# mir-group/pair_allegro

Measured on AMD Instinct MI355X. Metric: atom_steps_per_sec, higher is better.
Workload: dtype f32-equivalent (f16x2 split on the f16 matrix cores, f32 accumulate); 1 GPU; BASELINE config 4: 1000000-atom bulk Si (50^3 diamond cells), model S (l_max=1, U=32, S=64, 2 layers), r_max 5.0 A + skin 1.0 A, NVE dt=1 fs; grid=1x1x1, rebuilds=4, comm=serial, comm_transport=library/hosted/single-rank gather-scatter

## Files before the change

### pair_allegro_amd/csrc/fused.hip

```cpp
#include <hip/hip_runtime.h>

#include <cmath>
#include <algorithm>
#include <cstdio>
#include <cstdlib>
#include <cstring>
#include <type_traits>

#include "../../include/allegro_hip.h"
#include "engine.h"
#define AHIP_RING 4
#include "fused_common.h"
#include "fused_h.h"
#include "prims.h"

#ifndef AHIP_FUSED_PART
#define AHIP_FUSED_PART 0
#endif
namespace ahip {


[[maybe_unused]] static constexpr int MAX_TILE_SLOTS = 128;
static constexpr int MAXNL = 3;
static constexpr int STG_LD = 132;
// ... 23 lines not shown
  double *f, *eatom, *partial;
  long long *prof;
  float *dbg;
  float cp[6];
  int *err;
  double *vatom;
};

template <int NW, int NL = MAXNL> struct __attribute__((aligned(16))) Lds {
  static constexpr int SLOTS = 16 * NW;
  static constexpr int MAXA = NW == 4 ? 6 : 12;
  float stage[SLOTS * STG_LD];
  float env[NL][MAXA * ENV_LD];
  float denv[MAXA * ENV_LD];
  float tp[NL][5 * 32];
  float park[NW][8 * ROW];
  double eacc[MAXA];
  double virw[NW][6];
  int aoff[2][MAXA + 2];
  float rc[16];
  float scale[16], shift[16];
  float res[NL][2];
  int chunk[2];
};


__device__ __host__ constexpr int R_Z1TB() { return 0; }
__device__ __host__ constexpr int R_Z2TB() { return 4; }
__device__ __host__ constexpr int R_U0() { return 8; }
__device__ __host__ constexpr int R_W0() { return 12; }
__device__ __host__ constexpr int R_LSZ(int MD) { return 16 + 4 * MD; }
__device__ __host__ constexpr int R_LAYER(int kk, int MD = 2) { return 16 + R_LSZ(MD) * kk; }
__device__ __host__ constexpr int R_TOTAL(int NL, int MD = 2) { return 16 + R_LSZ(MD) * NL; }

static constexpr float C_S3 = 1.7320508075688772f;
static constexpr float C_P1 = 0.5773502691896258f;
static constexpr float C_P4 = 0.7071067811865476f;

typedef __bf16 bf16x8 __attribute__((ext_vector_type(8)));
struct Bop { u32x4 hi, mid, lo; };

__device__ __forceinline__ f32x4 mfma_b(u32x4 a, u32x4 b, f32x4 c) {
  return __builtin_amdgcn_mfma_f32_16x16x32_bf16(__builtin_bit_cast(bf16x8, a), __builtin_bit_cast(bf16x8, b), c, 0, 0, 0);
}
__device__ __forceinline__ void split2(float v0, float v1, unsigned &hi, unsigned &mid, unsigned &lo) {
  const unsigned a = __builtin_bit_cast(unsigned, v0), b = __builtin_bit_cast(unsigned, v1);
// ... 96 lines not shown
  const int fidx = tid & 127;
  for (int a = tid >> 7; a < na; a += NW / 2) {
    const int s0 = aoff[a], s1 = aoff[a + 1];
    float acc0 = 0.f, acc1 = 0.f, acc2 = 0.f, acc3 = 0.f;
    int sl = s0;
    for (; sl + 4 <= s1; sl += 4) {
      acc0 += lds.stage[sl * STG_LD + fidx];
      acc1 += lds.stage[(sl + 1) * STG_LD + fidx];
      acc2 += lds.stage[(sl + 2) * STG_LD + fidx];
      acc3 += lds.stage[(sl + 3) * STG_LD + fidx];
    }
    for (; sl < s1; ++sl) acc0 += lds.stage[sl * STG_LD + fidx];
    dst[a * ENV_LD + fidx] = scale * ((acc0 + acc1) + (acc2 + acc3));
  }
}
enum { PH_GEOM = 0, PH_TB, PH_EMB, PH_ENV, PH_TP, PH_MIX, PH_LAT, PH_OUT, PH_BLAT, PH_BMIX, PH_BTP, PH_BENV, PH_BEMB, PH_BTB, PH_FIN, PH_N };
#define PHASE(id) do { if (PROF) { long long _t = clock64(); pacc[id] += _t - tprev; tprev = _t; } } while (0)

template <int AR> struct RingT {
  int act = 1;
  f32x4 f[AR != 0 ? 1 : RING];
  u32x4 b[AR == 0 ? 1 : (AR == 1 ? RINGB : AR == 2 ? RINGB2 : RINGH)];
};
template <int AR, int KT, int NT, bool ACC, int RPI, class Epi>
__device__ __forceinline__ void lin(__amdgpu_buffer_rsrc_t W, int &wp, const f32x4 (&in)[KT], f32x4 (&out)[NT], int v16, RingT<AR> &ring, Epi epi) {
  if (!ring.act) {
    if constexpr (!ACC) {
#pragma unroll
      for (int t = 0; t < NT; ++t) out[t] = f32x4{0.f, 0.f, 0.f, 0.f};
    }
    return;
  }
  if constexpr (AR == 3) {
    static_assert(KT % 2 == 0, "K-steps are pairs of 16-feature tiles");
    Hop b[1][KT / 2], unused[1][NT / 2];
#pragma unroll
    for (int ks = 0; ks < KT / 2; ++ks) b[0][ks] = split_pair_h(in[2 * ks], in[2 * ks + 1]);
    Epi ep[1] = {epi};
    linear_h<1, KT / 2, NT, ACC, false, (4 * RPI) % RINGH, Epi>(W, wp, b, reinterpret_cast<f32x4 (&)[1][NT]>(out), unused, v16, ring.b, ep);
  } else if constexpr (AR != 0) {
    static_assert(KT % 2 == 0, "K-steps are pairs of 16-feature tiles");
    constexpr int NTERM = AR == 1 ? 3 : 2;
    Bop b[KT / 2], unused[NT / 2];
#pragma unroll
    for (int ks = 0; ks < KT / 2; ++ks) b[ks] = split_pair(in[2 * ks], in[2 * ks + 1]);
    linear_b<KT / 2, NT, ACC, false, (2 * NTERM * RPI) % RingB<NTERM>::N, Epi, NTERM>(W, wp, b, out, unused, v16, ring.b, epi);
  } else {
    linear_s<KT, NT, ACC, (4 * RPI) % RING, Epi>(W, wp, in, out, v16, ring.f, epi);
  }
}

template <int RPI, class Epi>
__device__ __forceinline__ void lin_m3(__amdgpu_buffer_rsrc_t W, int &wp, const f32x4 (&in0)[2], const f32x4 (&in1)[2], const f32x4 (&in2)[2], f32x4 (&out)[3][2], int v16,
                                       RingT<3> &ring, Epi (&epi)[3]) {
  if (!ring.act) {
#pragma unroll
    for (int q = 0; q < 3; ++q) { out[q][0] = f32x4{0.f, 0.f, 0.f, 0.f}; out[q][1] = f32x4{0.f, 0.f, 0.f, 0.f}; }
    return;
  }
  Hop b[3][1], unused[3][1];
  b[0][0] = split_pair_h(in0[0], in0[1]); b[1][0] = split_pair_h(in1[0], in1[1]); b[2][0] = split_pair_h(in2[0], in2[1]);
  linear_h<3, 1, 2, false, false, (4 * RPI) % RINGH, Epi>(W, wp, b, out, unused, v16, ring.b, epi);
}

struct TileIn {
  int a0, a1, e0, e1;
  float rx, ry, rz;
  int eii, jat, tt;
  int eoff;
};
__device__ __forceinline__ void tile_fetch(const FusedArgs &A, int tile, int ntiles, int s, int tid, TileIn &n) {
  n.a0 = n.a1 = n.e0 = n.e1 = 0;
  n.rx = 1.f; n.ry = 0.f; n.rz = 0.f;
  n.eii = 0; n.jat = 0; n.tt = 0; n.eoff = 0;
  if (tile >= ntiles) return;
  n.a0 = A.tile_a0[tile]; n.a1 = A.tile_a0[tile + 1]; n.e0 = A.tile_e0[tile]; n.e1 = A.tile_e0[tile + 1];
  const int e = n.e0 + s, na = n.a1 - n.a0;
  if (e < n.e1) {
    n.rx = A.rvec[3 * (size_t)e]; n.ry = A.rvec[3 * (size_t)e + 1]; n.rz = A.rvec[3 * (size_t)e + 2];
    n.eii = A.e_ii[e];
    n.jat = A.e_j[e];
    n.tt = A.e_tt[e];
  }
  if (tid <= na) n.eoff = A.eoff[n.a0 + tid];
}

template <int NW, bool PROF, int AR, bool TBT, int NLT, int MD = 2, bool VA = false, int RD = 1>
__global__ void __launch_bounds__(NW * 64, 2) k_fused(FusedArgs A) {
  constexpr int NTHREADS = NW * 64, MAXA = Lds<NW>::MAXA;
  constexpr bool SAVEZ = AR == 3;
  constexpr bool PARKV = true;
  constexpr bool STGROWS = true;
  constexpr int OZL = 4 + 4 * (MD - 1), OU = 4 + 4 * MD, OVIN = 8 + 4 * MD;
  static_assert(MD >= 1 && MD <= 3 && (MD == 2 || (AR == 3 && TBT)), "latent MLP depth 1 / 3: f16x2 instances with the two-body table only");
  static_assert(RD == 1 || (RD == 2 && AR == 3 && TBT && !PROF), "read-out depth 2: f16x2 instances with the two-body table only, not profiled");
  __shared__ Lds<NW, NLT> lds;
  const int tid = threadIdx.x, lane = tid & 63, j = lane & 15, g = lane >> 4, wave = tid >> 6;
  const int v16 = lane * 16;
  __amdgpu_buffer_rsrc_t SB, WB;
  {
    unsigned long long b = (unsigned long long)(A.scratch + (size_t)blockIdx.x * A.wg_scratch + (size_t)wave * A.wave_scratch);
    unsigned lo = __builtin_amdgcn_readfirstlane((unsigned)b), hi = __builtin_amdgcn_readfirstlane((unsigned)(b >> 32));
    SB = __builtin_amdgcn_make_buffer_rsrc((void *)(((unsigned long long)hi << 32) | lo), 0, (int)(A.wave_scratch * 4), 0x00020000);
    WB = __builtin_amdgcn_make_buffer_rsrc((void *)A.wbase, 0, A.wbytes, 0x00020000);
  }
  if (A.maxdeg_sel && ((*A.maxdeg_sel <= 64) != (NW == 4))) return;
  const float *__restrict__ Wb = A.wbase;
// ... 2 lines not shown
    lds.tp[k / 160][k % 160] = Wb[A.o_tpl + k] * (pth == 1 ? C_P1 : pth == 4 ? C_P4 : 1.f);
  }
  const int ntiles = *A.ntiles;
  constexpr int NL = NLT;
  double acc_part = 0.0;
  long long pacc[PH_N];
  long long tprev = 0;
  const long long t_clk0 = clock64(), t_wall0 = wall_clock64();
  if (PROF) {
#pragma unroll
    for (int k = 0; k < PH_N; ++k) pacc[k] = 0;
    tprev = clock64();
  }
  float *const pk = lds.park[wave];
  RingT<AR> ring;
  int wp = A.o_stream;
  if constexpr (AR != 0) ring_prime_b(WB, wp, v16, ring.b);
  else ring_prime(WB, wp, v16, ring.f);
  if (tid < MAXA) lds.eacc[tid] = 0.0;
  if (lane < 6) lds.virw[wave][lane] = 0.0;
  if (A.T <= 4 && tid < A.T * A.T) lds.rc[tid] = (float)A.rcut[tid];
  if (tid < A.T) { lds.scale[tid] = Wb[A.o_scale + tid]; lds.shift[tid] = Wb[A.o_shift + tid]; }
  if (tid < 2 * A.NL) lds.res[tid >> 1][tid & 1] = Wb[A.o_res[tid >> 1] + (tid & 1)];

  const int s = wave * 16 + j;
  float *const st = lds.stage + s * STG_LD;
  if (tid == 0) lds.chunk[0] = (int)atomicAdd(A.tile_counter, (unsigned)A.tchunk);
  __syncthreads();
  int par = 0, cpar = 0, ck = 0;
  int cbase = __builtin_amdgcn_readfirstlane(lds.chunk[0]);

  TileIn nx_;
  tile_fetch(A, cbase, ntiles, s, tid, nx_);

  for (;;) {
    const int tile = cbase + ck;
    if (tile >= ntiles) break;
    int claimed = 0;
    if (ck == 0 && tid == 0) claimed = (int)atomicAdd(A.tile_counter, (unsigned)A.tchunk);
    const int a0 = nx_.a0, a1 = nx_.a1, e0 = nx_.e0, e1 = nx_.e1;
    const int wact = __builtin_amdgcn_readfirstlane(e0 + wave * 16 < e1 ? 1 : 0);
    ring.act = wact;
    const int v16t = wact ? v16 : 0x7ffffff0;
    const int na = a1 - a0;
    par ^= 1;
    int *const aoffp = lds.aoff[par];
    const int e = e0 + s;
    const bool valid = e < e1;
    const float rx = nx_.rx, ry = nx_.ry, rz = nx_.rz;
    const int aloc = valid ? nx_.eii - a0 : 0, jat = nx_.jat, ti = nx_.tt >> 4, tj = nx_.tt & 15;
    if (tid <= na) aoffp[tid] = nx_.eoff - e0;
    const float d = sqrtf(rx * rx + ry * ry + rz * rz);
    const float inv = 1.f / d;
    const float nx = rx * inv, ny = ry * inv, nz = rz * inv;
    const float rc = A.T <= 4 ? lds.rc[ti * A.T + tj] : (float)A.rcut[ti * A.T + tj];
    const float xx = d / rc;
    float fc, dfc_dx;
    cutoff_poly_c(A.p, A.cp, xx, fc, dfc_dx);
    if (!valid) { fc = 0.f; dfc_dx = 0.f; }
    const float Y1 = C_S3 * ny, Y2 = C_S3 * nz, Y3 = C_S3 * nx;
    const float pref = 2.f / rc;
    const float PI = 3.14159265358979323846f;
    const float *const envrow = lds.env[0] + aloc * ENV_LD;
    const float *const denvrow = lds.denv + aloc * ENV_LD;
    PHASE(PH_GEOM);

    f32x4 x[4];
    float tb_t = 0.f, tb_invh = 0.f;
    if constexpr (TBT) {
      tb_invh = (float)A.tb_nk / rc;
      const float sft = d * tb_invh;
      const int kq = min((int)sft, A.tb_nk - 1);
// ... 16 lines not shown
      {
        const float *pt = Wb + A.o_pair + (size_t)(ti * A.T + tj) * 64;
#pragma unroll
        for (int t = 0; t < 4; ++t) z[t] = *(const f32x4 *)(pt + 16 * t + 4 * g);
      }
      f32x4 bfin[2];
#pragma unroll
      for (int r = 0; r < 4; ++r) {
        const float n = (float)(4 * g + r + 1);
        bfin[0][r] = g < 2 ? pref * __builtin_amdgcn_sinf(0.5f * n * xx) * inv * fc : 0.f;
        bfin[1][r] = 0.f;
      }
      lin<AR, 2, 4, true, 0>(WB, wp, bfin, z, v16t, ring, EpiSiluSaveD{SB, R_Z1TB(), v16t});
      lin<AR, 4, 4, false, 0>(WB, wp, z, z2, v16t, ring, EpiSiluSaveD{SB, R_Z2TB(), v16t});
      lin<AR, 4, 4, false, 0>(WB, wp, z2, x, v16t, ring, EpiSaveScale{{SB, R_U0(), v16t}, fc});
    }
    PHASE(PH_TB);
    {
      f32x4 w0[4];
      lin<AR, 4, 4, false, 0>(WB, wp, x, w0, v16t, ring, EpiSavePark{{SB, R_W0(), v16t}, pk, 0, lane});
    }
    if (ck == 0 && tid == 0) lds.chunk[cpar ^ 1] = claimed;
    __syncthreads();
    PHASE(PH_EMB);

    f32x4 zr[2];
#pragma unroll
    for (int kk = 0; kk < NL; ++kk) {
      const bool last = (kk == NL - 1);
      const int RL = R_LAYER(kk, MD);
      float *const envk = lds.env[0] + kk * (MAXA * ENV_LD);
      f32x4 V[4][2];
      {
        f32x4 om[4];
        lin<AR, 4, 4, false, 0>(WB, wp, x, om, v16t, ring, EpiSaveFrom2{{SB, RL + 0, v16t}});
#pragma unroll
        for (int t = 0; t < 2; ++t) {
          float *sp = st + 16 * t + 4 * g;
          *(f32x4 *)(sp) = om[t];
          *(f32x4 *)(sp + 32) = om[2 + t] * Y1;
          *(f32x4 *)(sp + 64) = om[2 + t] * Y2;
          *(f32x4 *)(sp + 96) = om[2 + t] * Y3;
        }
        __syncthreads();
        reduce_stage(lds, aoffp, envk, na, A.cenv, tid);
        __syncthreads();
// ... 20 lines not shown
#pragma unroll
        for (int t = 0; t < 2; ++t) {
          const int b = 16 * t + 4 * g;
          const f32x4 e0v = *(const f32x4 *)(en + b), e1v = *(const f32x4 *)(en + 32 + b), e2v = *(const f32x4 *)(en + 64 + b),
                      e3v = *(const f32x4 *)(en + 96 + b);
          const f32x4 v0 = V[0][t], v1 = V[1][t], v2 = V[2][t], v3 = V[3][t];
          Vp[0][t] = *(const f32x4 *)(tp + b) * v0 * e0v + *(const f32x4 *)(tp + 32 + b) * (v1 * e1v + v2 * e2v + v3 * e3v);
          if (!last) {
            const f32x4 p2 = *(const f32x4 *)(tp + 64 + b), p3 = *(const f32x4 *)(tp + 96 + b), c4 = *(const f32x4 *)(tp + 128 + b);
            const f32x4 p2v0 = p2 * v0, p3e0 = p3 * e0v;
            Vp[1][t] = p2v0 * e1v + p3e0 * v1 + c4 * (v2 * e3v - v3 * e2v);
            Vp[2][t] = p2v0 * e2v + p3e0 * v2 + c4 * (v3 * e1v - v1 * e3v);
            Vp[3][t] = p2v0 * e3v + p3e0 * v3 + c4 * (v1 * e2v - v2 * e1v);
          }
          __builtin_amdgcn_sched_barrier(0);
        }
      }
      PHASE(PH_TP);
      if (!last) {
        f32x4 o2[2];
        if constexpr (AR == 3) {
          f32x4 o3[3][2];
          if (PARKV && kk + 1 == NL - 1) {
            lin<AR, 2, 2, false, 0>(WB, wp, Vp[0], o2, v16t, ring, EpiPark{pk, 0, lane});
            EpiPark ep[3] = {EpiPark{pk, 2, lane}, EpiPark{pk, 4, lane}, EpiPark{pk, 6, lane}};
            lin_m3<1>(WB, wp, Vp[1], Vp[2], Vp[3], o3, v16t, ring, ep);
          } else {
            lin<AR, 2, 2, false, 0>(WB, wp, Vp[0], o2, v16t, ring, EpiSavePark{{SB, R_LAYER(kk + 1, MD) + OVIN + 0, v16t}, pk, 0, lane});
            EpiSavePark ep[3] = {EpiSavePark{{SB, R_LAYER(kk + 1, MD) + OVIN + 2, v16t}, pk, 2, lane}, EpiSavePark{{SB, R_LAYER(kk + 1, MD) + OVIN + 4, v16t}, pk, 4, lane},
                                 EpiSavePark{{SB, R_LAYER(kk + 1, MD) + OVIN + 6, v16t}, pk, 6, lane}};
            lin_m3<1>(WB, wp, Vp[1], Vp[2], Vp[3], o3, v16t, ring, ep);
          }
        } else if (PARKV && kk + 1 == NL - 1) {
          lin<AR, 2, 2, false, 0>(WB, wp, Vp[0], o2, v16t, ring, EpiPark{pk, 0, lane});
          lin<AR, 2, 2, false, 1>(WB, wp, Vp[1], o2, v16t, ring, EpiPark{pk, 2, lane});
          lin<AR, 2, 2, false, 2>(WB, wp, Vp[2], o2, v16t, ring, EpiPark{pk, 4, lane});
          lin<AR, 2, 2, false, 3>(WB, wp, Vp[3], o2, v16t, ring, EpiPark{pk, 6, lane});
        } else {
          lin<AR, 2, 2, false, 0>(WB, wp, Vp[0], o2, v16t, ring, EpiSavePark{{SB, R_LAYER(kk + 1, MD) + OVIN + 0, v16t}, pk, 0, lane});
          lin<AR, 2, 2, false, 1>(WB, wp, Vp[1], o2, v16t, ring, EpiSavePark{{SB, R_LAYER(kk + 1, MD) + OVIN + 2, v16t}, pk, 2, lane});
          lin<AR, 2, 2, false, 2>(WB, wp, Vp[2], o2, v16t, ring, EpiSavePark{{SB, R_LAYER(kk + 1, MD) + OVIN + 4, v16t}, pk, 4, lane});
          lin<AR, 2, 2, false, 3>(WB, wp, Vp[3], o2, v16t, ring, EpiSavePark{{SB, R_LAYER(kk + 1, MD) + OVIN + 6, v16t}, pk, 6, lane});
        }
      }
      PHASE(PH_MIX);
      {
        f32x4 cat[6], z[4], z2[4];
        cat[0] = x[0]; cat[1] = x[1]; cat[2] = x[2]; cat[3] = x[3]; cat[4] = Vp[0][0]; cat[5] = Vp[0][1];
        const bool stg = STGROWS && last;
        float *const sq = st + 4 * g;
#define AHIP_HIDDEN(KT, IN, OUT, H) do { \
          if (stg && (H) >= MD - 1) { \
            if (SAVEZ && (H) == MD) lin<AR, KT, 4, false, 0>(WB, wp, IN, OUT, v16t, ring, EpiSiluSaveZL{sq, 4}); \
            else lin<AR, KT, 4, false, 0>(WB, wp, IN, OUT, v16t, ring, EpiSiluSaveDL{sq, (H) == MD ? 4 : 0}); \
// ... 18 lines not shown
          zr[0] = ra * za[0] + rbf * up[0]; zr[1] = ra * za[1] + rbf * up[1];
        }
      }
      PHASE(PH_LAT);
    }

    f32x4 upre[4], zt[4], w0h[2];
#pragma unroll
    for (int t = 0; t < 2; ++t) if (!SAVEZ) upre[t] = bload(SB, v16t, (R_LAYER(NL - 1, MD) + OU + t) * ROW * 4);
    if (!STGROWS) load_rows<4>(SB, R_LAYER(NL - 1, MD) + OZL, zt, v16t);
    __builtin_amdgcn_sched_barrier(0);
    f32x4 zr2[2];
    if constexpr (RD == 2) {
      f32x4 hr[2];
#pragma unroll
      for (int t = 0; t < 2; ++t)
#pragma unroll
        for (int r = 0; r < 4; ++r) hr[t][r] = silu1(zr[t][r]);
      lin<AR, 2, 2, false, 0>(WB, wp, hr, zr2, v16t, ring, EpiNone{});
    }
    f32x4 (&zo)[2] = RD == 2 ? zr2 : zr;
    f32x4 wo1[2];
#pragma unroll
    for (int t = 0; t < 2; ++t) wo1[t] = *(const f32x4 *)(Wb + A.o_out1 + 16 * t + 4 * g);
    float eps = 0.f;
#pragma unroll
    for (int t = 0; t < 2; ++t)
#pragma unroll
      for (int r = 0; r < 4; ++r) eps += silu1(zo[t][r]) * wo1[t][r];
    eps = gsum(eps);
    asm volatile("" : "+v"(eps));

    float bsc = 1.f;
    if constexpr (AR == 3) {
      int bex;
      (void)frexpf(lds.scale[ti] * A.cenv, &bex);
      bex = min(max(bex, -100), 100);
      bsc = ldexpf(1.f, -bex);
      if (g == 0) st[128] = ldexpf(1.f, bex);
    }
    const float deps = valid ? lds.scale[ti] * A.cenv * bsc : 0.f;
    f32x4 dx[4];
    f32x4 dzr[2];
#pragma unroll
    for (int t = 0; t < 2; ++t)
#pragma unroll
      for (int r = 0; r < 4; ++r) dzr[t][r] = deps * wo1[t][r] * dsilu1(zo[t][r]);
// ... 93 lines not shown
        for (int t = 0; t < 4; ++t) dx[t] += dcat[t];
        dVp[0][0] = dcat[4]; dVp[0][1] = dcat[5];
      }
      if (kk == 0) {
#pragma unroll
        for (int t = 0; t < 2; ++t) {
          Vk[0][t] = W0b[t];
          Vk[1][t] = W0b[2 + t] * Y1; Vk[2][t] = W0b[2 + t] * Y2; Vk[3][t] = W0b[2 + t] * Y3;
        }
      }
      if (PARKV && last && kk > 0) {
#pragma unroll
        for (int lm = 0; lm < 4; ++lm)
#pragma unroll
          for (int t = 0; t < 2; ++t) Vk[lm][t] = park_load(pk, 2 * lm + t, lane);
      }
      f32x4 om1[2];
      load_rows<2>(SB, RL + 2, om1, v16t);
      __builtin_amdgcn_sched_barrier(0);
      PHASE(PH_BLAT);
      if (!last) {
        f32x4 in2[2], o2[2];
        in2[0] = park_load(pk, 0, lane); in2[1] = park_load(pk, 1, lane);
        lin<AR, 2, 2, false, 0>(WB, wp, in2, o2, v16t, ring, EpiNone{});
        dVp[0][0] += o2[0]; dVp[0][1] += o2[1];
        if constexpr (AR == 3) {
          f32x4 i1[2] = {park_load(pk, 2, lane), park_load(pk, 3, lane)}, i2[2] = {park_load(pk, 4, lane), park_load(pk, 5, lane)},
                i3[2] = {park_load(pk, 6, lane), park_load(pk, 7, lane)};
          f32x4 o3[3][2];
          EpiNone ep[3];
          lin_m3<1>(WB, wp, i1, i2, i3, o3, v16t, ring, ep);
#pragma unroll
          for (int q = 0; q < 3; ++q) { dVp[1 + q][0] = o3[q][0]; dVp[1 + q][1] = o3[q][1]; }
        } else {
          in2[0] = park_load(pk, 2, lane); in2[1] = park_load(pk, 3, lane);
          lin<AR, 2, 2, false, 1>(WB, wp, in2, dVp[1], v16t, ring, EpiNone{});
          in2[0] = park_load(pk, 4, lane); in2[1] = park_load(pk, 5, lane);
          lin<AR, 2, 2, false, 2>(WB, wp, in2, dVp[2], v16t, ring, EpiNone{});
          in2[0] = park_load(pk, 6, lane); in2[1] = park_load(pk, 7, lane);
          lin<AR, 2, 2, false, 3>(WB, wp, in2, dVp[3], v16t, ring, EpiNone{});
        }
      }
      __builtin_amdgcn_sched_barrier(0);
      PHASE(PH_BMIX);
      {
        const float *en = envrow + kk * (MAXA * ENV_LD);
        const float *tp = lds.tp[kk];
#pragma unroll
        for (int t = 0; t < 2; ++t) {
          const int b = 16 * t + 4 * g;
          const f32x4 e0v = *(const f32x4 *)(en + b), e1v = *(const f32x4 *)(en + 32 + b), e2v = *(const f32x4 *)(en + 64 + b),
                      e3v = *(const f32x4 *)(en + 96 + b);
          const f32x4 v0 = Vk[0][t], v1 = Vk[1][t], v2 = Vk[2][t], v3 = Vk[3][t];
          const f32x4 g0 = dVp[0][t];
          const f32x4 q0 = *(const f32x4 *)(tp + b) * g0, q1 = *(const f32x4 *)(tp + 32 + b) * g0;
          f32x4 a0v = q0 * e0v, a1v = q1 * e1v, a2v = q1 * e2v, a3v = q1 * e3v;
          f32x4 b0v = q0 * v0, b1v = q1 * v1, b2v = q1 * v2, b3v = q1 * v3;
// ... 33 lines not shown
                      d3 = *(const f32x4 *)(denvrow + 96 + b);
          dom[t] = d0;
          dom[2 + t] = d1 * Y1 + d2 * Y2 + d3 * Y3;
          const f32x4 p1 = d1 * om1[t], p2 = d2 * om1[t], p3 = d3 * om1[t];
          dY1 += (p1[0] + p1[1]) + (p1[2] + p1[3]); dY2 += (p2[0] + p2[1]) + (p2[2] + p2[3]); dY3 += (p3[0] + p3[1]) + (p3[2] + p3[3]);
          __builtin_amdgcn_sched_barrier(0);
        }
        asm volatile("" : "+v"(dY1), "+v"(dY2), "+v"(dY3));
        if (kk > 0) {
          if (!SAVEZ) load_rows<4>(SB, R_LAYER(kk - 1, MD) + OU, upre, v16t);
          load_rows<4>(SB, R_LAYER(kk - 1, MD) + OZL, zt, v16t);
        } else {
          if constexpr (!TBT) {
            load_rows<4>(SB, R_U0(), upre, v16t);
            load_rows<4>(SB, R_Z2TB(), zt, v16t);
          } else load_rows<4>(SB, R_Z1TB(), zt, v16t);
          load_rows<2>(SB, R_W0() + 2, w0h, v16t);
        }
        __builtin_amdgcn_sched_barrier(0);
        lin<AR, 4, 4, true, 0>(WB, wp, dom, dx, v16t, ring, EpiNone{});
      }
      PHASE(PH_BENV);
    }
    {
      const int ntile = (ck + 1 == A.tchunk) ? __builtin_amdgcn_readfirstlane(lds.chunk[cpar ^ 1]) : tile + 1;
      tile_fetch(A, ntile, ntiles, s, tid, nx_);
    }
    f32x4 zt1b[4];
    if constexpr (!TBT) load_rows<4>(SB, R_Z1TB(), zt1b, v16t);
    __builtin_amdgcn_sched_barrier(0);
    {
      f32x4 dw0[4];
#pragma unroll
      for (int t = 0; t < 2; ++t) {
        const f32x4 d0 = park_load(pk, 0 + t, lane), d1 = park_load(pk, 2 + t, lane), d2 = park_load(pk, 4 + t, lane), d3 = park_load(pk, 6 + t, lane);
        dw0[t] = d0;
        dw0[2 + t] = d1 * Y1 + d2 * Y2 + d3 * Y3;
#pragma unroll
        for (int r = 0; r < 4; ++r) { dY1 += d1[r] * w0h[t][r]; dY2 += d2[r] * w0h[t][r]; dY3 += d3[r] * w0h[t][r]; }
      }
      asm volatile("" : "+v"(dY1), "+v"(dY2), "+v"(dY3));
      lin<AR, 4, 4, true, 0>(WB, wp, dw0, dx, v16t, ring, EpiNone{});
      if constexpr (TBT) wp = A.o_stream;
    }
    PHASE(PH_BEMB);
    float dd_part = 0.f;
    if constexpr (TBT) {
      f32x4 accv = dx[0] * zt[0];
#pragma unroll
      for (int t = 1; t < 4; ++t) accv += dx[t] * zt[t];
// ... 24 lines not shown
    }
    PHASE(PH_BTB);
    {
      const float ibs = AR == 3 ? st[128] : 1.f;
      const float dfc_tot = gsum(dfc_part) * ibs;
      const float dd = dfc_tot * (dfc_dx / rc) + gsum(dd_part) * ibs;
      const float y1 = gsum(dY1) * ibs, y2 = gsum(dY2) * ibs, y3 = gsum(dY3) * ibs;
      const float Gx = C_S3 * y3, Gy = C_S3 * y1, Gz = C_S3 * y2;
      float rxe = rx, rye = ry, rze = rz;
      asm volatile("" : "+v"(rxe), "+v"(rye), "+v"(rze));
      const float inve = 1.f / sqrtf(rxe * rxe + rye * rye + rze * rze);
      const float nxe = rxe * inve, nye = rye * inve, nze = rze * inve;
      const float gn = Gx * nxe + Gy * nye + Gz * nze;
      const float gx = dd * nxe + (Gx - gn * nxe) * inve;
      const float gy = dd * nye + (Gy - gn * nye) * inve;
      const float gz = dd * nze + (Gz - gn * nze) * inve;
      if (A.dbg && valid && g == 0) {
        float *dp = A.dbg + 8 * (size_t)e;
        dp[0] = gx; dp[1] = gy; dp[2] = gz; dp[3] = dd; dp[4] = dfc_tot; dp[5] = y1; dp[6] = y2; dp[7] = y3;
      }
#if !defined(ABL_NOW) && !defined(ABL_NOROWS) && !defined(ABL_NOROWLD) && !defined(ABL_NOROWST)
      if (AR == 3 && valid && !(fabsf(gx) + fabsf(gy) + fabsf(gz) + fabsf(eps) < 3.0e38f)) *A.err = 1;
#endif
      if (g == 0) {
        st[0] = valid ? gx : 0.f; st[1] = valid ? gy : 0.f; st[2] = valid ? gz : 0.f; st[3] = valid ? eps : 0.f;
        if (valid) {
#ifndef ABL_NOATOM
          atomicAdd(&A.f[3 * (size_t)jat], -(double)gx);
          atomicAdd(&A.f[3 * (size_t)jat + 1], -(double)gy);
          atomicAdd(&A.f[3 * (size_t)jat + 2], -(double)gz);
#endif
        }
      }
      float w6[6] = {-rx * gx, -ry * gy, -rz * gz, -0.5f * (rx * gy + ry * gx), -0.5f * (rx * gz + rz * gx), -0.5f * (ry * gz + rz * gy)};
#pragma unroll
      for (int c = 0; c < 6; ++c) w6[c] = valid ? w6[c] : 0.f;
#pragma unroll
      for (int c = 0; c < 6; ++c) {
#pragma unroll
        for (int off = 8; off > 0; off >>= 1) w6[c] += __shfl_xor(w6[c], off, 64);
      }
      if (lane < 6) {
        const float mine = lane == 0 ? w6[0] : lane == 1 ? w6[1] : lane == 2 ? w6[2] : lane == 3 ? w6[3] : lane == 4 ? w6[4] : w6[5];
        lds.virw[wave][lane] += (double)mine;
      }
      if constexpr (VA) vatom_scatter(A.vatom, jat, g, valid, rx, ry, rz, gx, gy, gz);
    }
    int tidf = tid;
    asm volatile("" : "+v"(tidf));
    const int caf = tidf >> 4;
    int2 cil = make_int2(0, 0);
    if (caf < na) cil = A.centre[a0 + caf];
    __syncthreads();
    {
      const int col = tidf & 3, part = (tidf >> 2) & 3;
      float sum = 0.f;
      if (caf < na)
        for (int sl = aoffp[caf] + part; sl < aoffp[caf + 1]; sl += 4) sum += lds.stage[sl * STG_LD + col];
      sum += __shfl_xor(sum, 4, 64);
      sum += __shfl_xor(sum, 8, 64);
      if (caf < na && part == 0) {
        if (col < 3) atomicAdd(&A.f[3 * (size_t)cil.x + col], (double)sum);
        else {
          const float ei = lds.scale[cil.y] * (sum * A.cenv) + lds.shift[cil.y];
          if (A.eatom) A.eatom[cil.x] = (double)ei;
          lds.eacc[caf] += (double)ei;
        }
      }
    }
    PHASE(PH_FIN);
    if (++ck == A.tchunk) { ck = 0; cpar ^= 1; cbase = __builtin_amdgcn_readfirstlane(lds.chunk[cpar]); }
  }
  __syncthreads();
  if (tid == 0) {
    for (int a = 0; a < MAXA; ++a) acc_part += lds.eacc[a];
  } else if (tid >= 64 && tid < 70) {
    for (int w = 0; w < NW; ++w) acc_part += lds.virw[w][tid - 64];
  }
  if (PROF && lane == 0) {
#pragma unroll
    for (int k = 0; k < PH_N; ++k) atomicAdd((unsigned long long *)&A.prof[k], (unsigned long long)pacc[k]);
  }
  if (A.prof && tid == 0) {
    long long *o = A.prof + PH_N + 4 * (size_t)blockIdx.x;
    o[0] = clock64() - t_clk0;
    o[1] = t_wall0;
    o[2] = wall_clock64();
    o[3] = ((long long)__builtin_amdgcn_s_getreg((20 << 0) | (0 << 6) | (31 << 11)) << 32) | (unsigned)__builtin_amdgcn_s_getreg((4 << 0) | (0 << 6) | (31 << 11));
  }
  if (tid == 0) A.partial[7 * (size_t)blockIdx.x] = acc_part;
  if (tid >= 64 && tid < 70) A.partial[7 * (size_t)blockIdx.x + 1 + (tid - 64)] = acc_part;
}


void fused_launch_bf16(int nw, bool prof, int arith, bool tbt, int grid, hipStream_t s, const FusedArgs &A);
void fused_launch_f16(int nw, bool prof, int md, int grid, hipStream_t s, const FusedArgs &A);
void fused_launch_f16_rd2(int nw, int md, int grid, hipStream_t s, const FusedArgs &A);
#if AHIP_FUSED_PART == 3
void fused_launch_f16_rd2(int nw, int md, int grid, hipStream_t s, const FusedArgs &A) {
  dispatch<Choices<4, 8>, Choices<1, 2, 3>, Choices<1, 3, 2>, Choices<VAR_VA, VAR_PLAIN>>([&](auto nw, auto nl, auto md, auto var) {
    hipLaunchKernelGGL((k_fused<nw, false, 3, true, nl, md, var == VAR_VA, 2>), dim3(grid), dim3(nw * 64), 0, s, A);
  }, nw, A.NL, md, fused_variant(A.vatom, false));
}
#endif
#if AHIP_FUSED_PART == 2
void fused_launch_f16(int nw, bool prof, int md, int grid, hipStream_t s, const FusedArgs &A) {
#ifdef AHIP_ASM_ONLY
#ifndef AHIP_ASM_NW
#define AHIP_ASM_NW 4
#endif
  hipLaunchKernelGGL((k_fused<AHIP_ASM_NW, false, 3, true, 2, 2>), dim3(grid), dim3(AHIP_ASM_NW * 64), 0, s, A);
#else
  dispatch<Choices<4, 8>, Choices<1, 2, 3>, Choices<1, 3, 2>, Variants>([&](auto nw, auto nl, auto md, auto var) {
    if constexpr (var != VAR_PROF || md == 2) hipLaunchKernelGGL((k_fused<nw, var == VAR_PROF, 3, true, nl, md, var == VAR_VA>), dim3(grid), dim3(nw * 64), 0, s, A);
// ... 422 lines not shown
```

### pair_allegro_amd/csrc/fused_h.h

```cpp
#pragma once
#include <cstring>

#include "fused_common.h"

namespace ahip {

typedef _Float16 f16x2 __attribute__((ext_vector_type(2)));
typedef _Float16 f16x8 __attribute__((ext_vector_type(8)));
typedef float f32x2 __attribute__((ext_vector_type(2)));
struct Hop { u32x4 hi, lo; };
static constexpr float H_LO_SCALE = 2048.f, H_LO_INV = 1.f / 2048.f;
static constexpr int RINGH = 8;

__device__ __forceinline__ f32x4 mfma_h(u32x4 a, u32x4 b, f32x4 c) {
  return __builtin_amdgcn_mfma_f32_16x16x32_f16(__builtin_bit_cast(f16x8, a), __builtin_bit_cast(f16x8, b), c, 0, 0, 0);
}
__device__ __forceinline__ void split2_h(float v0, float v1, unsigned &hi, unsigned &lo) {
  const f32x2 v = {v0, v1};
  const f16x2 h = __builtin_convertvector(v, f16x2);
  const f32x2 r = (v - __builtin_convertvector(h, f32x2)) * H_LO_SCALE;
  const f16x2 l = __builtin_convertvector(r, f16x2);
  hi = __builtin_bit_cast(unsigned, h);
  lo = __builtin_bit_cast(unsigned, l);
}
__device__ __forceinline__ Hop split_pair_h(const f32x4 &t0, const f32x4 &t1) {
  Hop b;
  unsigned h, l;
  split2_h(t0[0], t0[1], h, l); b.hi[0] = h; b.lo[0] = l;
  split2_h(t0[2], t0[3], h, l); b.hi[1] = h; b.lo[1] = l;
  split2_h(t1[0], t1[1], h, l); b.hi[2] = h; b.lo[2] = l;
  split2_h(t1[2], t1[3], h, l); b.hi[3] = h; b.lo[3] = l;
  return b;
}

__device__ __forceinline__ void ring_prime_h(__amdgpu_buffer_rsrc_t W, int wp, int v16, u32x4 (&ring)[RINGH]) {
  int wo = wp * 4;
  pin_s(wo);
#pragma unroll
  for (int j = 0; j < RINGH; ++j) ring[j] = __builtin_bit_cast(u32x4, bload_w(W, v16 + (j & 3) * 1024, wo + (j >> 2) * 4096));
}

template <class E> __device__ __forceinline__ auto epi_apply2(E &e, int ot, int r, f32x2 v, int) -> decltype(e.apply2(ot, r, v)) { return e.apply2(ot, r, v); }
template <class E> __device__ __forceinline__ f32x2 epi_apply2(E &e, int ot, int r, f32x2 v, long) { return f32x2{e.apply(ot, r, v[0]), e.apply(ot, r + 1, v[1])}; }

template <int G, int KS, int NT, bool ACC, bool SPLIT, int RP, class Epi>
__device__ __forceinline__ void linear_h(__amdgpu_buffer_rsrc_t W, int &wp, const Hop (&in)[G][KS], f32x4 (&out)[G][NT], Hop (&outb)[G][NT / 2],
                                         int v16, u32x4 (&ring)[RINGH], Epi (&epi)[G]) {
  static_assert(NT % 2 == 0, "output tiles are processed in pairs");
  constexpr int RB = RINGH, NF = 4, NP = NT / 2, NSTEP = NP * KS, NS = NF * NSTEP;
  constexpr int MF = 6 * G;
  f32x4 ah[G][2], ac[G][2], prev[G][2];
  int wo = (wp + RB * 256) * 4;
  pin_s(wo);
#pragma unroll
  for (int s = 0; s < NSTEP; ++s) {
    const int p = s / KS, ks = s % KS;
    if (ks == 0) {
#pragma unroll
      for (int g = 0; g < G; ++g)
#pragma unroll
        for (int hh = 0; hh < 2; ++hh) {
          ah[g][hh] = ACC ? out[g][2 * p + hh] : f32x4{0.f, 0.f, 0.f, 0.f};
          ac[g][hh] = f32x4{0.f, 0.f, 0.f, 0.f};
        }
    }
    u32x4 a[NF];
#pragma unroll
    for (int i = 0; i < NF; ++i) {
      a[i] = ring[(RP + NF * s + i) % RB];
      ring[(RP + NF * s + i) % RB] = __builtin_bit_cast(u32x4, bload_w(W, v16 + i * 1024, wo));
    }
    wo += NF * 1024;
    pin_s(wo);
#pragma unroll
    for (int m = 0; m < 3; ++m) {
#pragma unroll
      for (int hh = 0; hh < 2; ++hh) {
#pragma unroll
        for (int g = 0; g < G; ++g) {
          if (m == 0) ac[g][hh] = mfma_h(a[2 + hh], in[g][ks].hi, ac[g][hh]);
          else if (m == 1) ac[g][hh] = mfma_h(a[hh], in[g][ks].lo, ac[g][hh]);
          else ah[g][hh] = mfma_h(a[hh], in[g][ks].hi, ah[g][hh]);
          if (p > 0) {
            const int idx = ks * MF + (m * 2 + hh) * G + g, tot = KS * MF, NE = 4 * G;
            const int e0 = (idx * NE + tot - 1) / tot, e1 = ((idx + 1) * NE + tot - 1) / tot;
#pragma unroll
            for (int e = 0; e < NE; ++e)
              if (e >= e0 && e < e1) {
                const int eg = e / 4, th = (e % 4) / 2, r = 2 * (e % 2), ot = 2 * (p - 1) + th;
                const f32x2 y = epi_apply2(epi[eg], ot, r, f32x2{prev[eg][th][r], prev[eg][th][r + 1]}, 0);
                out[eg][ot][r] = y[0]; out[eg][ot][r + 1] = y[1];
                if (e % 4 == 3) {
                  epi[eg].flush(2 * (p - 1));
                  if (SPLIT) outb[eg][p - 1] = split_pair_h(out[eg][2 * (p - 1)], out[eg][2 * (p - 1) + 1]);
                }
              }
          }
          __builtin_amdgcn_sched_barrier(0);
        }
      }
    }
    if (ks == KS - 1) {
#pragma unroll
      for (int g = 0; g < G; ++g) {
        const f32x4 r0 = ac[g][0] * H_LO_INV + ah[g][0], r1 = ac[g][1] * H_LO_INV + ah[g][1];
        epi[g].tile_done(2 * p, r0);
        epi[g].tile_done(2 * p + 1, r1);
        if (p == NP - 1) {
#pragma unroll
          for (int r = 0; r < 4; r += 2) {
            const f32x2 y0 = epi_apply2(epi[g], 2 * p, r, f32x2{r0[r], r0[r + 1]}, 0), y1 = epi_apply2(epi[g], 2 * p + 1, r, f32x2{r1[r], r1[r + 1]}, 0);
            out[g][2 * p][r] = y0[0]; out[g][2 * p][r + 1] = y0[1]; out[g][2 * p + 1][r] = y1[0]; out[g][2 * p + 1][r + 1] = y1[1];
          }
          epi[g].flush(2 * p);
          if (SPLIT) outb[g][p] = split_pair_h(out[g][2 * p], out[g][2 * p + 1]);
        } else { prev[g][0] = r0; prev[g][1] = r1; }
      }
    }
    __builtin_amdgcn_sched_barrier(0);
  }
  wp += NS * 256;
  pin_s(wp);
}
// ... 41 lines not shown
```

Baseline: 27.51 million atom-steps/s.

## Prefetch tile lists via buffer loads, merge mix linears, and defer weight-ring refills

Several independent changes are bundled. Next-tile edge and offset lists are now fetched with raw buffer loads bounded by per-tile resources, and tile bounds are read through constant address space earlier in the loop. The centre-atom index load moves ahead of the barrier. The two mix linears are merged behind a single activity branch. Short f16 linear_h calls now refill the weight ring interleaved with the MFMAs instead of up front. Output weights are cached in LDS, and the tile-counter atomic is rewritten as an explicit relaxed agent-scope add. The aim is to hide global-load latency and reduce branch and scheduling overhead, at the cost of more live registers and more complex ordering.

Result: faster. 27.83 million atom-steps/s, median of 6 (+1.1%).

```diff
diff --git a/pair_allegro_amd/csrc/fused.hip b/pair_allegro_amd/csrc/fused.hip
--- a/pair_allegro_amd/csrc/fused.hip
+++ b/pair_allegro_amd/csrc/fused.hip
@@ -69,6 +69,7 @@
   float scale[16], shift[16];
   float res[NL][2];
   int chunk[2];
+  float wo1[32];
 };
 
 
@@ -211,9 +212,9 @@
   f32x4 f[AR != 0 ? 1 : RING];
   u32x4 b[AR == 0 ? 1 : (AR == 1 ? RINGB : AR == 2 ? RINGB2 : RINGH)];
 };
-template <int AR, int KT, int NT, bool ACC, int RPI, class Epi>
+template <int AR, int KT, int NT, bool ACC, int RPI, bool BR = true, class Epi>
 __device__ __forceinline__ void lin(__amdgpu_buffer_rsrc_t W, int &wp, const f32x4 (&in)[KT], f32x4 (&out)[NT], int v16, RingT<AR> &ring, Epi epi) {
-  if (!ring.act) {
+  if (BR && !ring.act) {
     if constexpr (!ACC) {
 #pragma unroll
       for (int t = 0; t < NT; ++t) out[t] = f32x4{0.f, 0.f, 0.f, 0.f};
@@ -226,7 +227,7 @@
 #pragma unroll
     for (int ks = 0; ks < KT / 2; ++ks) b[0][ks] = split_pair_h(in[2 * ks], in[2 * ks + 1]);
     Epi ep[1] = {epi};
-    linear_h<1, KT / 2, NT, ACC, false, (4 * RPI) % RINGH, Epi>(W, wp, b, reinterpret_cast<f32x4 (&)[1][NT]>(out), unused, v16, ring.b, ep);
+    linear_h<1, KT / 2, NT, ACC, false, (4 * RPI) % RINGH, Epi, true>(W, wp, b, reinterpret_cast<f32x4 (&)[1][NT]>(out), unused, v16, ring.b, ep);
   } else if constexpr (AR != 0) {
     static_assert(KT % 2 == 0, "K-steps are pairs of 16-feature tiles");
     constexpr int NTERM = AR == 1 ? 3 : 2;
@@ -239,17 +240,29 @@
   }
 }
 
-template <int RPI, class Epi>
+template <int RPI, bool BR = true, class Epi>
 __device__ __forceinline__ void lin_m3(__amdgpu_buffer_rsrc_t W, int &wp, const f32x4 (&in0)[2], const f32x4 (&in1)[2], const f32x4 (&in2)[2], f32x4 (&out)[3][2], int v16,
                                        RingT<3> &ring, Epi (&epi)[3]) {
-  if (!ring.act) {
+  if (BR && !ring.act) {
 #pragma unroll
     for (int q = 0; q < 3; ++q) { out[q][0] = f32x4{0.f, 0.f, 0.f, 0.f}; out[q][1] = f32x4{0.f, 0.f, 0.f, 0.f}; }
     return;
   }
   Hop b[3][1], unused[3][1];
   b[0][0] = split_pair_h(in0[0], in0[1]); b[1][0] = split_pair_h(in1[0], in1[1]); b[2][0] = split_pair_h(in2[0], in2[1]);
-  linear_h<3, 1, 2, false, false, (4 * RPI) % RINGH, Epi>(W, wp, b, out, unused, v16, ring.b, epi);
+  linear_h<3, 1, 2, false, false, (4 * RPI) % RINGH, Epi, true>(W, wp, b, out, unused, v16, ring.b, epi);
+}
+template <class Epi0, class Epi3>
+__device__ __forceinline__ void lin_mix(__amdgpu_buffer_rsrc_t W, int &wp, const f32x4 (&in0)[2], const f32x4 (&in1)[2], const f32x4 (&in2)[2], const f32x4 (&in3)[2], f32x4 (&out0)[2],
+                                        f32x4 (&out)[3][2], int v16, RingT<3> &ring, Epi0 epi0, Epi3 (&epi)[3]) {
+  if (!ring.act) {
+    out0[0] = f32x4{0.f, 0.f, 0.f, 0.f}; out0[1] = f32x4{0.f, 0.f, 0.f, 0.f};
+#pragma unroll
+    for (int q = 0; q < 3; ++q) { out[q][0] = f32x4{0.f, 0.f, 0.f, 0.f}; out[q][1] = f32x4{0.f, 0.f, 0.f, 0.f}; }
+    return;
+  }
+  lin<3, 2, 2, false, 0, false>(W, wp, in0, out0, v16, ring, epi0);
+  lin_m3<1, false>(W, wp, in1, in2, in3, out, v16, ring, epi);
 }
 
 struct TileIn {
@@ -258,20 +271,31 @@
   int eii, jat, tt;
   int eoff;
 };
-__device__ __forceinline__ void tile_fetch(const FusedArgs &A, int tile, int ntiles, int s, int tid, TileIn &n) {
-  n.a0 = n.a1 = n.e0 = n.e1 = 0;
-  n.rx = 1.f; n.ry = 0.f; n.rz = 0.f;
-  n.eii = 0; n.jat = 0; n.tt = 0; n.eoff = 0;
-  if (tile >= ntiles) return;
-  n.a0 = A.tile_a0[tile]; n.a1 = A.tile_a0[tile + 1]; n.e0 = A.tile_e0[tile]; n.e1 = A.tile_e0[tile + 1];
-  const int e = n.e0 + s, na = n.a1 - n.a0;
-  if (e < n.e1) {
-    n.rx = A.rvec[3 * (size_t)e]; n.ry = A.rvec[3 * (size_t)e + 1]; n.rz = A.rvec[3 * (size_t)e + 2];
-    n.eii = A.e_ii[e];
-    n.jat = A.e_j[e];
-    n.tt = A.e_tt[e];
-  }
-  if (tid <= na) n.eoff = A.eoff[n.a0 + tid];
+struct TileBounds { int a0, a1, e0, e1; };
+typedef const __attribute__((address_space(4))) int *cint_p;
+__device__ __forceinline__ TileBounds tile_bounds(const FusedArgs &A, int tile, int ntiles) {
+  const int tc = max(min(tile, ntiles - 1), 0);
+  const cint_p ta = (cint_p)(unsigned long long)A.tile_a0, te = (cint_p)(unsigned long long)A.tile_e0;
+  TileBounds b = {ta[tc], ta[tc + 1], te[tc], te[tc + 1]};
+  if (tile >= ntiles) b = TileBounds{0, 0, 0, 0};
+  return b;
+}
+__device__ __forceinline__ __amdgpu_buffer_rsrc_t list_rsrc(const void *base, long long first_byte, int bytes) {
+  return __builtin_amdgcn_make_buffer_rsrc((void *)((unsigned long long)base + (unsigned long long)first_byte), 0, bytes, 0x00020000);
+}
+__device__ __forceinline__ void tile_fetch(const FusedArgs &A, const TileBounds &b, int s, int tid, TileIn &n) {
+  n.a0 = b.a0; n.a1 = b.a1; n.e0 = b.e0; n.e1 = b.e1;
+  const int ne = b.e1 - b.e0, na = b.a1 - b.a0;
+  const int eb = b.e0 & 3;
+  const __amdgpu_buffer_rsrc_t RV = list_rsrc(A.rvec, 12ll * b.e0, 12 * ne), EI = list_rsrc(A.e_ii, 4ll * b.e0, 4 * ne), EJ = list_rsrc(A.e_j, 4ll * b.e0, 4 * ne),
+                               ET = list_rsrc(A.e_tt, b.e0 - eb, ne + eb), EO = list_rsrc(A.eoff, 4ll * b.a0, na > 0 ? 4 * (na + 1) : 0);
+  n.rx = __builtin_bit_cast(float, __builtin_amdgcn_raw_buffer_load_b32(RV, 12 * s, 0, 0));
+  n.ry = __builtin_bit_cast(float, __builtin_amdgcn_raw_buffer_load_b32(RV, 12 * s + 4, 0, 0));
+  n.rz = __builtin_bit_cast(float, __builtin_amdgcn_raw_buffer_load_b32(RV, 12 * s + 8, 0, 0));
+  n.eii = (int)__builtin_amdgcn_raw_buffer_load_b32(EI, 4 * s, 0, 0);
+  n.jat = (int)__builtin_amdgcn_raw_buffer_load_b32(EJ, 4 * s, 0, 0);
+  n.tt = (int)__builtin_amdgcn_raw_buffer_load_b8(ET, s + eb, 0, 0);
+  n.eoff = (int)__builtin_amdgcn_raw_buffer_load_b32(EO, 4 * tid, 0, 0);
 }
 
 template <int NW, bool PROF, int AR, bool TBT, int NLT, int MD = 2, bool VA = false, int RD = 1>
@@ -320,6 +344,7 @@
   if (A.T <= 4 && tid < A.T * A.T) lds.rc[tid] = (float)A.rcut[tid];
   if (tid < A.T) { lds.scale[tid] = Wb[A.o_scale + tid]; lds.shift[tid] = Wb[A.o_shift + tid]; }
   if (tid < 2 * A.NL) lds.res[tid >> 1][tid & 1] = Wb[A.o_res[tid >> 1] + (tid & 1)];
+  if (tid >= 64 && tid < 96) lds.wo1[tid - 64] = Wb[A.o_out1 + tid - 64];
 
   const int s = wave * 16 + j;
   float *const st = lds.stage + s * STG_LD;
@@ -329,13 +354,18 @@
   int cbase = __builtin_amdgcn_readfirstlane(lds.chunk[0]);
 
   TileIn nx_;
-  tile_fetch(A, cbase, ntiles, s, tid, nx_);
+  tile_fetch(A, tile_bounds(A, cbase, ntiles), s, tid, nx_);
+  asm volatile("" : "+v"(nx_.rx), "+v"(nx_.ry), "+v"(nx_.rz), "+v"(nx_.eii), "+v"(nx_.jat), "+v"(nx_.tt), "+v"(nx_.eoff));
 
   for (;;) {
     const int tile = cbase + ck;
     if (tile >= ntiles) break;
     int claimed = 0;
-    if (ck == 0 && tid == 0) claimed = (int)atomicAdd(A.tile_counter, (unsigned)A.tchunk);
+    if (ck == 0 && tid == 0) {
+      unsigned long long tcnt = (unsigned long long)A.tile_counter;
+      asm volatile("" : "+v"(tcnt));
+      claimed = (int)__hip_atomic_fetch_add((__attribute__((address_space(1))) unsigned int *)tcnt, (unsigned)A.tchunk, __ATOMIC_RELAXED, __HIP_MEMORY_SCOPE_AGENT);
+    }
     const int a0 = nx_.a0, a1 = nx_.a1, e0 = nx_.e0, e1 = nx_.e1;
     const int wact = __builtin_amdgcn_readfirstlane(e0 + wave * 16 < e1 ? 1 : 0);
     ring.act = wact;
@@ -345,7 +375,7 @@
     int *const aoffp = lds.aoff[par];
     const int e = e0 + s;
     const bool valid = e < e1;
-    const float rx = nx_.rx, ry = nx_.ry, rz = nx_.rz;
+    const float rx = valid ? nx_.rx : 1.f, ry = nx_.ry, rz = nx_.rz;
     const int aloc = valid ? nx_.eii - a0 : 0, jat = nx_.jat, ti = nx_.tt >> 4, tj = nx_.tt & 15;
     if (tid <= na) aoffp[tid] = nx_.eoff - e0;
     const float d = sqrtf(rx * rx + ry * ry + rz * rz);
@@ -408,6 +438,7 @@
     }
     if (ck == 0 && tid == 0) lds.chunk[cpar ^ 1] = claimed;
     __syncthreads();
+    const TileBounds nb_ = tile_bounds(A, (ck + 1 == A.tchunk) ? __builtin_amdgcn_readfirstlane(lds.chunk[cpar ^ 1]) : tile + 1, ntiles);
     PHASE(PH_EMB);
 
     f32x4 zr[2];
@@ -474,14 +505,12 @@
         if constexpr (AR == 3) {
           f32x4 o3[3][2];
           if (PARKV && kk + 1 == NL - 1) {
-            lin<AR, 2, 2, false, 0>(WB, wp, Vp[0], o2, v16t, ring, EpiPark{pk, 0, lane});
             EpiPark ep[3] = {EpiPark{pk, 2, lane}, EpiPark{pk, 4, lane}, EpiPark{pk, 6, lane}};
-            lin_m3<1>(WB, wp, Vp[1], Vp[2], Vp[3], o3, v16t, ring, ep);
+            lin_mix(WB, wp, Vp[0], Vp[1], Vp[2], Vp[3], o2, o3, v16t, ring, EpiPark{pk, 0, lane}, ep);
           } else {
-            lin<AR, 2, 2, false, 0>(WB, wp, Vp[0], o2, v16t, ring, EpiSavePark{{SB, R_LAYER(kk + 1, MD) + OVIN + 0, v16t}, pk, 0, lane});
             EpiSavePark ep[3] = {EpiSavePark{{SB, R_LAYER(kk + 1, MD) + OVIN + 2, v16t}, pk, 2, lane}, EpiSavePark{{SB, R_LAYER(kk + 1, MD) + OVIN + 4, v16t}, pk, 4, lane},
                                  EpiSavePark{{SB, R_LAYER(kk + 1, MD) + OVIN + 6, v16t}, pk, 6, lane}};
-            lin_m3<1>(WB, wp, Vp[1], Vp[2], Vp[3], o3, v16t, ring, ep);
+            lin_mix(WB, wp, Vp[0], Vp[1], Vp[2], Vp[3], o2, o3, v16t, ring, EpiSavePark{{SB, R_LAYER(kk + 1, MD) + OVIN + 0, v16t}, pk, 0, lane}, ep);
           }
         } else if (PARKV && kk + 1 == NL - 1) {
           lin<AR, 2, 2, false, 0>(WB, wp, Vp[0], o2, v16t, ring, EpiPark{pk, 0, lane});
@@ -546,7 +575,7 @@
     f32x4 (&zo)[2] = RD == 2 ? zr2 : zr;
     f32x4 wo1[2];
 #pragma unroll
-    for (int t = 0; t < 2; ++t) wo1[t] = *(const f32x4 *)(Wb + A.o_out1 + 16 * t + 4 * g);
+    for (int t = 0; t < 2; ++t) wo1[t] = *(const f32x4 *)(lds.wo1 + 16 * t + 4 * g);
     float eps = 0.f;
 #pragma unroll
     for (int t = 0; t < 2; ++t)
@@ -686,17 +715,18 @@
       if (!last) {
         f32x4 in2[2], o2[2];
         in2[0] = park_load(pk, 0, lane); in2[1] = park_load(pk, 1, lane);
-        lin<AR, 2, 2, false, 0>(WB, wp, in2, o2, v16t, ring, EpiNone{});
-        dVp[0][0] += o2[0]; dVp[0][1] += o2[1];
         if constexpr (AR == 3) {
           f32x4 i1[2] = {park_load(pk, 2, lane), park_load(pk, 3, lane)}, i2[2] = {park_load(pk, 4, lane), park_load(pk, 5, lane)},
                 i3[2] = {park_load(pk, 6, lane), park_load(pk, 7, lane)};
           f32x4 o3[3][2];
           EpiNone ep[3];
-          lin_m3<1>(WB, wp, i1, i2, i3, o3, v16t, ring, ep);
+          lin_mix(WB, wp, in2, i1, i2, i3, o2, o3, v16t, ring, EpiNone{}, ep);
+          dVp[0][0] += o2[0]; dVp[0][1] += o2[1];
 #pragma unroll
           for (int q = 0; q < 3; ++q) { dVp[1 + q][0] = o3[q][0]; dVp[1 + q][1] = o3[q][1]; }
         } else {
+          lin<AR, 2, 2, false, 0>(WB, wp, in2, o2, v16t, ring, EpiNone{});
+          dVp[0][0] += o2[0]; dVp[0][1] += o2[1];
           in2[0] = park_load(pk, 2, lane); in2[1] = park_load(pk, 3, lane);
           lin<AR, 2, 2, false, 1>(WB, wp, in2, dVp[1], v16t, ring, EpiNone{});
           in2[0] = park_load(pk, 4, lane); in2[1] = park_load(pk, 5, lane);
@@ -776,10 +806,10 @@
       }
       PHASE(PH_BENV);
     }
-    {
-      const int ntile = (ck + 1 == A.tchunk) ? __builtin_amdgcn_readfirstlane(lds.chunk[cpar ^ 1]) : tile + 1;
-      tile_fetch(A, ntile, ntiles, s, tid, nx_);
-    }
+    tile_fetch(A, nb_, s, tid, nx_);
+    int tidc = tid;
+    asm volatile("" : "+v"(tidc));
+    auto cil_ = __builtin_amdgcn_raw_buffer_load_b64(list_rsrc(A.centre, 8ll * a0, 8 * na), (tidc >> 4) * 8, 0, 0);
     f32x4 zt1b[4];
     if constexpr (!TBT) load_rows<4>(SB, R_Z1TB(), zt1b, v16t);
     __builtin_amdgcn_sched_barrier(0);
@@ -850,6 +880,7 @@
 #if !defined(ABL_NOW) && !defined(ABL_NOROWS) && !defined(ABL_NOROWLD) && !defined(ABL_NOROWST)
       if (AR == 3 && valid && !(fabsf(gx) + fabsf(gy) + fabsf(gz) + fabsf(eps) < 3.0e38f)) *A.err = 1;
 #endif
+      asm volatile("" : "+v"(nx_.rx), "+v"(nx_.ry), "+v"(nx_.rz), "+v"(nx_.eii), "+v"(nx_.jat), "+v"(nx_.tt), "+v"(nx_.eoff), "+v"(cil_));
       if (g == 0) {
         st[0] = valid ? gx : 0.f; st[1] = valid ? gy : 0.f; st[2] = valid ? gz : 0.f; st[3] = valid ? eps : 0.f;
         if (valid) {
@@ -877,9 +908,8 @@
     int tidf = tid;
     asm volatile("" : "+v"(tidf));
     const int caf = tidf >> 4;
-    int2 cil = make_int2(0, 0);
-    if (caf < na) cil = A.centre[a0 + caf];
     __syncthreads();
+    const int2 cil = make_int2((int)cil_[0], (int)cil_[1]);
     {
       const int col = tidf & 3, part = (tidf >> 2) & 3;
       float sum = 0.f;
@@ -900,10 +930,12 @@
     if (++ck == A.tchunk) { ck = 0; cpar ^= 1; cbase = __builtin_amdgcn_readfirstlane(lds.chunk[cpar]); }
   }
   __syncthreads();
-  if (tid == 0) {
+  int tide = tid;
+  asm volatile("" : "+v"(tide));
+  if (tide == 0) {
     for (int a = 0; a < MAXA; ++a) acc_part += lds.eacc[a];
-  } else if (tid >= 64 && tid < 70) {
-    for (int w = 0; w < NW; ++w) acc_part += lds.virw[w][tid - 64];
+  } else if (tide >= 64 && tide < 70) {
+    for (int w = 0; w < NW; ++w) acc_part += lds.virw[w][tide - 64];
   }
   if (PROF && lane == 0) {
 #pragma unroll
@@ -916,8 +948,8 @@
     o[2] = wall_clock64();
     o[3] = ((long long)__builtin_amdgcn_s_getreg((20 << 0) | (0 << 6) | (31 << 11)) << 32) | (unsigned)__builtin_amdgcn_s_getreg((4 << 0) | (0 << 6) | (31 << 11));
   }
-  if (tid == 0) A.partial[7 * (size_t)blockIdx.x] = acc_part;
-  if (tid >= 64 && tid < 70) A.partial[7 * (size_t)blockIdx.x + 1 + (tid - 64)] = acc_part;
+  if (tide == 0) A.partial[7 * (size_t)blockIdx.x] = acc_part;
+  if (tide >= 64 && tide < 70) A.partial[7 * (size_t)blockIdx.x + 1 + (tide - 64)] = acc_part;
 }
 
 
diff --git a/pair_allegro_amd/csrc/fused_h.h b/pair_allegro_amd/csrc/fused_h.h
--- a/pair_allegro_amd/csrc/fused_h.h
+++ b/pair_allegro_amd/csrc/fused_h.h
@@ -43,12 +43,16 @@
 template <class E> __device__ __forceinline__ auto epi_apply2(E &e, int ot, int r, f32x2 v, int) -> decltype(e.apply2(ot, r, v)) { return e.apply2(ot, r, v); }
 template <class E> __device__ __forceinline__ f32x2 epi_apply2(E &e, int ot, int r, f32x2 v, long) { return f32x2{e.apply(ot, r, v[0]), e.apply(ot, r + 1, v[1])}; }
 
-template <int G, int KS, int NT, bool ACC, bool SPLIT, int RP, class Epi>
+template <int G, int KS, int NT, bool ACC, bool SPLIT, int RP, class Epi, bool LATE_OK = false>
 __device__ __forceinline__ void linear_h(__amdgpu_buffer_rsrc_t W, int &wp, const Hop (&in)[G][KS], f32x4 (&out)[G][NT], Hop (&outb)[G][NT / 2],
                                          int v16, u32x4 (&ring)[RINGH], Epi (&epi)[G]) {
   static_assert(NT % 2 == 0, "output tiles are processed in pairs");
   constexpr int RB = RINGH, NF = 4, NP = NT / 2, NSTEP = NP * KS, NS = NF * NSTEP;
   constexpr int MF = 6 * G;
+#ifndef AHIP_LATE_STEPS
+#define AHIP_LATE_STEPS 2
+#endif
+  constexpr bool LATE = LATE_OK && NSTEP <= AHIP_LATE_STEPS;
   f32x4 ah[G][2], ac[G][2], prev[G][2];
   int wo = (wp + RB * 256) * 4;
   pin_s(wo);
@@ -66,12 +70,18 @@
     }
     u32x4 a[NF];
 #pragma unroll
-    for (int i = 0; i < NF; ++i) {
-      a[i] = ring[(RP + NF * s + i) % RB];
-      ring[(RP + NF * s + i) % RB] = __builtin_bit_cast(u32x4, bload_w(W, v16 + i * 1024, wo));
+    for (int i = 0; i < NF; ++i) a[i] = ring[(RP + NF * s + i) % RB];
+    if (!LATE) {
+#pragma unroll
+      for (int q = 0; q < NF; ++q) {
+        const int i = LATE_OK ? (q + 2) % NF : q;
+        ring[(RP + NF * s + i) % RB] = __builtin_bit_cast(u32x4, bload_w(W, v16 + i * 1024, wo));
+      }
     }
-    wo += NF * 1024;
-    pin_s(wo);
+    if (!LATE) {
+      wo += NF * 1024;
+      pin_s(wo);
+    }
 #pragma unroll
     for (int m = 0; m < 3; ++m) {
 #pragma unroll
@@ -81,6 +91,10 @@
           if (m == 0) ac[g][hh] = mfma_h(a[2 + hh], in[g][ks].hi, ac[g][hh]);
           else if (m == 1) ac[g][hh] = mfma_h(a[hh], in[g][ks].lo, ac[g][hh]);
           else ah[g][hh] = mfma_h(a[hh], in[g][ks].hi, ah[g][hh]);
+          if (LATE && g == G - 1 && m != 1) {
+            const int i = m == 0 ? 2 + hh : hh;
+            ring[(RP + NF * s + i) % RB] = __builtin_bit_cast(u32x4, bload_w(W, v16 + i * 1024, wo));
+          }
           if (p > 0) {
             const int idx = ks * MF + (m * 2 + hh) * G + g, tot = KS * MF, NE = 4 * G;
             const int e0 = (idx * NE + tot - 1) / tot, e1 = ((idx + 1) * NE + tot - 1) / tot;
@@ -99,6 +113,10 @@
           __builtin_amdgcn_sched_barrier(0);
         }
       }
+    }
+    if (LATE) {
+      wo += NF * 1024;
+      pin_s(wo);
     }
     if (ks == KS - 1) {
 #pragma unroll
```
